# ethz-asl/laser_slam

Measured on NVIDIA H100. Metric: ICP registrations/s (131072-pt scan vs 524288-pt map, 30 iterations), higher is better.
Workload: dtype f32

## Files before the change

laser_slam_b200/csrc/ls_grid.cuh:

```cuda
#pragma once
#include <cfloat>
#include <climits>
#include <cstring>

#include <vector_types.h>
#include <vector_functions.h>

#include "ls_math.cuh"

#define LS_FB 8
#define LS_FB3 (LS_FB * LS_FB * LS_FB)
#define LS_PYR_LEVELS 7

namespace ls {

struct Entry {
  uint32_t start;
  int32_t meta;
};

struct Grid {
  float org[3];
  float H0, H1;
  float inv0, inv1;
  int dim[3];
  int n_cells0;
  float margin;
  float mu[3];
  int m;
  int leaf_split;
  int n_tab1;
  int overflow;
  int n_pyr;
  int pdim[LS_PYR_LEVELS + 1][3];
  int poff[LS_PYR_LEVELS + 1];
  int n_pyr_cells;
};

struct GridView {
  const Entry* top;
  const Entry* tab1;
  const float4* pts;
  const unsigned long long* pyr;
  const unsigned long long* topmask;
};

struct Best {
  float d2;
  int idx;
  int pos;
  LS_HD float bound() const { return d2; }
  LS_HD void offer(float d, int i, int p) {
    if (d < d2 || (d == d2 && i < idx)) {
      d2 = d;
      idx = i;
      pos = p;
    }
  }
  LS_HD void offer_pt(float d, const float4& c, int p);
};

#define LS_KNN_MAX 16
struct TopK {
  float d[LS_KNN_MAX];
  int id[LS_KNN_MAX];
  int k;
  float cap;
  LS_HD void reset(int kk) {
    k = kk;
    cap = INFINITY;
    for (int j = 0; j < LS_KNN_MAX; ++j) { d[j] = INFINITY; id[j] = INT_MAX; }
  }
  LS_HD float bound() const { return fminf(d[k - 1], cap); }
  LS_HD void offer(float dist, int i, int) {
    if (dist > cap || !(dist < d[k - 1] || (dist == d[k - 1] && i < id[k - 1]))) return;
    for (int j = 0; j < k; ++j)
      if (id[j] == i) return;
    int j = k - 1;
    while (j > 0 && (dist < d[j - 1] || (dist == d[j - 1] && i < id[j - 1]))) {
      d[j] = d[j - 1];
      id[j] = id[j - 1];
      --j;
    }
    d[j] = dist;
    id[j] = i;
  }
  LS_HD void offer_pt(float dist, const float4& c, int p);
};

#if defined(LS_SIM_COUNTERS) && !defined(__CUDA_ARCH__)
extern thread_local long long ls_sim_cand, ls_sim_entries, ls_sim_steps;
#define LS_CNT_CAND() (++ls_sim_cand)
#define LS_CNT_ENTRY() (++ls_sim_entries)
#define LS_CNT_STEP() (++ls_sim_steps)
#else
#define LS_CNT_CAND() ((void)0)
#define LS_CNT_ENTRY() ((void)0)
#define LS_CNT_STEP() ((void)0)
#endif

#if defined(__CUDA_ARCH__)
LS_HD float4 ld_pt(const float4* p) { return __ldg(p); }
LS_HD Entry ld_entry(const Entry* e) {
  const int2 v = __ldg(reinterpret_cast<const int2*>(e));
  Entry r;
  r.start = (uint32_t)v.x;
  r.meta = v.y;
  return r;
}
LS_HD int f2i(float f) { return __float_as_int(f); }
LS_HD float i2f(int i) { return __int_as_float(i); }
LS_HD float4 ld_state4(const float4* p) { return __ldcg(p); }
LS_HD void st_state4(float4* p, const float4 v) { __stcg(p, v); }
LS_HD unsigned long long ld_mask(const unsigned long long* p) { return __ldg(p); }
LS_HD unsigned long long ld_rows(const unsigned long long* p) { return __ldg(p); }
LS_HD int ctz64(unsigned long long m) { return __ffsll((long long)m) - 1; }
#else
LS_HD float4 ld_pt(const float4* p) { LS_CNT_CAND(); return *p; }
LS_HD Entry ld_entry(const Entry* e) { LS_CNT_ENTRY(); return *e; }
LS_HD int f2i(float f) { int i; std::memcpy(&i, &f, 4); return i; }
LS_HD float i2f(int i) { float f; std::memcpy(&f, &i, 4); return f; }
LS_HD float4 ld_state4(const float4* p) { return *p; }
LS_HD void st_state4(float4* p, const float4 v) { *p = v; }
LS_HD unsigned long long ld_mask(const unsigned long long* p) { LS_CNT_ENTRY(); return *p; }
LS_HD unsigned long long ld_rows(const unsigned long long* p) { return *p; }
LS_HD int ctz64(unsigned long long m) { return __builtin_ctzll(m); }
#endif

LS_HD int coord_top(float v, float o, float inv, int n) {
  float t = floorf((v - o) * inv);
  t = fminf(fmaxf(t, 0.0f), (float)(n - 1));
  return (int)t;
}
LS_HD int coord_sub(float v, float lo, float inv) {
  float t = floorf((v - lo) * inv);
  t = fminf(fmaxf(t, 0.0f), (float)(LS_FB - 1));
  return (int)t;
}
LS_HD float cell_lo(float o, int c, float H) { return o + (float)c * H; }

LS_HD float gap(float q, float lo, float hi, float m) {
  const float a = (lo - m) - q;
  const float b = q - (hi + m);
  return fmaxf(0.0f, fmaxf(a, b));
}

#define LS_SHRINK 0.999999f

LS_HD float ball_radius(float best_d2, float margin) { return sqrtf(best_d2) * 1.000001f + margin; }

LS_HD void Best::offer_pt(float d, const float4& c, int p) { offer(d, f2i(c.w), p); }
LS_HD void TopK::offer_pt(float dist, const float4& c, int p) { offer(dist, f2i(c.w), p); }
template <class Acc>
LS_HD void consider_pt(const float4 p, int pos, float qx, float qy, float qz, Acc& b) {
  b.offer_pt(dist2(qx, qy, qz, p.x, p.y, p.z), p, pos);
}
template <class Acc>
LS_HD void consider(const float4* pts, int pos, float qx, float qy, float qz, Acc& b) {
  consider_pt(ld_pt(pts + pos), pos, qx, qy, qz, b);
}

template <class Acc>
LS_HD void scan_range(const float4* pts, uint32_t a, uint32_t e, float qx, float qy, float qz, Acc& b) {
  uint32_t pos = a;
  for (; pos + 4 <= e; pos += 4) {
    LS_CNT_STEP();
    const float4 p0 = ld_pt(pts + pos), p1 = ld_pt(pts + pos + 1), p2 = ld_pt(pts + pos + 2), p3 = ld_pt(pts + pos + 3);
    consider_pt(p0, (int)pos, qx, qy, qz, b);
    consider_pt(p1, (int)pos + 1, qx, qy, qz, b);
    consider_pt(p2, (int)pos + 2, qx, qy, qz, b);
    consider_pt(p3, (int)pos + 3, qx, qy, qz, b);
  }
  if (pos < e) LS_CNT_STEP();
  for (; pos < e; ++pos) consider(pts, (int)pos, qx, qy, qz, b);
}

template <class Acc>
LS_HD void visit_fine(const Grid& g, const Entry* tab, unsigned long long rows, float lox, float loy, float loz,
                      const float4* pts, float qx, float qy, float qz, Acc& b) {
  const float R = ball_radius(b.bound(), g.margin);
  const int x0 = coord_sub(qx - R, lox, g.inv1), x1 = coord_sub(qx + R, lox, g.inv1);
  const int y0 = coord_sub(qy - R, loy, g.inv1), y1 = coord_sub(qy + R, loy, g.inv1);
  const int z0 = coord_sub(qz - R, loz, g.inv1), z1 = coord_sub(qz + R, loz, g.inv1);
  for (int z = z0; z <= z1; ++z) {
    const float gz = gap(qz, cell_lo(loz, z, g.H1), cell_lo(loz, z + 1, g.H1), g.margin);
    const float gz2 = gz * gz;
    if (gz2 * LS_SHRINK > b.bound()) continue;
    const Entry* row = tab + (z * LS_FB + y0) * LS_FB;
    for (int y = y0; y <= y1; ++y, row += LS_FB) {
      if (!((rows >> (z * LS_FB + y)) & 1ull)) continue;
      const float gy = gap(qy, cell_lo(loy, y, g.H1), cell_lo(loy, y + 1, g.H1), g.margin);
      const float lb = gy * gy + gz2;
      if (lb * LS_SHRINK > b.bound()) continue;
      LS_CNT_STEP();
      const Entry e0 = ld_entry(row + x0);
      const Entry e1 = ld_entry(row + x1);
      scan_range(pts, e0.start, e1.start + (uint32_t)e1.meta, qx, qy, qz, b);
    }
  }
}

template <class Acc>
LS_HD void visit_top_entry(const Grid& g, const GridView& v, const Entry e, unsigned long long rows, float cx, float cy,
                           float cz, float qx, float qy, float qz, Acc& b) {
  if (e.meta > 0) {
    scan_range(v.pts, e.start, e.start + (uint32_t)e.meta, qx, qy, qz, b);
  } else if (e.meta < 0) {
    visit_fine(g, v.tab1 + (size_t)(~e.meta) * LS_FB3, rows, cx, cy, cz, v.pts, qx, qy, qz, b);
  }
}
template <class Acc>
LS_HD void visit_top_cell(const Grid& g, const GridView& v, int x, int y, int z, float cx, float cy, float cz, float qx,
                          float qy, float qz, Acc& b) {
  LS_CNT_STEP();
  const size_t ci = ((size_t)z * g.dim[1] + y) * g.dim[0] + x;
  const Entry e = ld_entry(v.top + ci);
  const unsigned long long rows = ld_rows(v.topmask + ci);
  visit_top_entry(g, v, e, rows, cx, cy, cz, qx, qy, qz, b);
}

template <class Acc>
LS_HDN void pyramid_query(const Grid& g, const GridView& v, float qx, float qy, float qz, Acc& b) {
  int lvl[LS_PYR_LEVELS + 1], bx[LS_PYR_LEVELS + 1], by[LS_PYR_LEVELS + 1], bz[LS_PYR_LEVELS + 1];
  unsigned long long mk[LS_PYR_LEVELS + 1];
  const int* td = g.pdim[g.n_pyr];
  const int n_top = td[0] * td[1] * td[2];
  for (int t = 0; t < n_top; ++t) {
    int sp = 0;
    lvl[0] = g.n_pyr;
    bx[0] = (t % td[0]) * 4;
    by[0] = ((t / td[0]) % td[1]) * 4;
    bz[0] = (t / (td[0] * td[1])) * 4;
    mk[0] = ld_mask(v.pyr + g.poff[g.n_pyr] + t);
    while (sp >= 0) {
      if (mk[sp] == 0ull) { --sp; continue; }
      const int bit = ctz64(mk[sp]);
      mk[sp] &= mk[sp] - 1ull;
      LS_CNT_STEP();
      const int cl = lvl[sp] - 1;
      const int cx = bx[sp] + (bit & 3), cy = by[sp] + ((bit >> 2) & 3), cz = bz[sp] + (bit >> 4);
      const float Hc = g.H0 * (float)(1 << (2 * cl));
      const float lx = cell_lo(g.org[0], cx, Hc), ly = cell_lo(g.org[1], cy, Hc), lz = cell_lo(g.org[2], cz, Hc);
      const float gx = gap(qx, lx, cell_lo(g.org[0], cx + 1, Hc), g.margin);
      const float gy = gap(qy, ly, cell_lo(g.org[1], cy + 1, Hc), g.margin);
      const float gz = gap(qz, lz, cell_lo(g.org[2], cz + 1, Hc), g.margin);
      const float lb = gx * gx + (gy * gy + gz * gz);
      if (lb * LS_SHRINK > b.bound()) continue;
      if (cl == 0) {
        visit_top_cell(g, v, cx, cy, cz, lx, ly, lz, qx, qy, qz, b);
      } else {
        ++sp;
        lvl[sp] = cl;
        bx[sp] = cx * 4; by[sp] = cy * 4; bz[sp] = cz * 4;
        mk[sp] = ld_mask(v.pyr + g.poff[cl] + ((size_t)cz * g.pdim[cl][1] + cy) * g.pdim[cl][0] + cx);
      }
    }
  }
}

template <class Acc>
LS_HD void ball_query(const Grid& g, const GridView& v, float qx, float qy, float qz, Acc& b) {
  const float R = ball_radius(b.bound(), g.margin);
  const int x0 = coord_top(qx - R, g.org[0], g.inv0, g.dim[0]), x1 = coord_top(qx + R, g.org[0], g.inv0, g.dim[0]);
  const int y0 = coord_top(qy - R, g.org[1], g.inv0, g.dim[1]), y1 = coord_top(qy + R, g.org[1], g.inv0, g.dim[1]);
  const int z0 = coord_top(qz - R, g.org[2], g.inv0, g.dim[2]), z1 = coord_top(qz + R, g.org[2], g.inv0, g.dim[2]);
  if ((x1 - x0 + 1) * (y1 - y0 + 1) * (z1 - z0 + 1) > 27 && g.n_pyr > 0) {
    pyramid_query(g, v, qx, qy, qz, b);
    return;
  }
  for (int z = z0; z <= z1; ++z) {
    const float cz = cell_lo(g.org[2], z, g.H0);
    const float gz = gap(qz, cz, cell_lo(g.org[2], z + 1, g.H0), g.margin);
    const float gz2 = gz * gz;
    if (gz2 * LS_SHRINK > b.bound()) continue;
    for (int y = y0; y <= y1; ++y) {
      const float cy = cell_lo(g.org[1], y, g.H0);
      const float gy = gap(qy, cy, cell_lo(g.org[1], y + 1, g.H0), g.margin);
      const float lbyz = gy * gy + gz2;
      if (lbyz * LS_SHRINK > b.bound()) continue;
      for (int x = x0; x <= x1; ++x) {
        const float cx = cell_lo(g.org[0], x, g.H0);
        const float gx = gap(qx, cx, cell_lo(g.org[0], x + 1, g.H0), g.margin);
        const float lb = gx * gx + lbyz;
        if (lb * LS_SHRINK > b.bound()) continue;
        visit_top_cell(g, v, x, y, z, cx, cy, cz, qx, qy, qz, b);
      }
    }
  }
}

LS_HDN void seed_query(const Grid& g, const GridView& v, float qx, float qy, float qz, Best& b) {
  const int cx = coord_top(qx, g.org[0], g.inv0, g.dim[0]);
  const int cy = coord_top(qy, g.org[1], g.inv0, g.dim[1]);
  const int cz = coord_top(qz, g.org[2], g.inv0, g.dim[2]);
  const Entry e = ld_entry(v.top + ((size_t)cz * g.dim[1] + cy) * g.dim[0] + cx);
  if (e.meta == 0) {
    int X = 0, Y = 0, Z = 0;
    const int* td = g.pdim[g.n_pyr];
    const int n_top = td[0] * td[1] * td[2];
    if (n_top > 1) {
      const float Ht = g.H0 * (float)(1 << (2 * g.n_pyr));
      float best_lb = INFINITY;
      for (int t = 0; t < n_top; ++t) {
        if (ld_mask(v.pyr + g.poff[g.n_pyr] + t) == 0ull) continue;
        const int tx = t % td[0], ty = (t / td[0]) % td[1], tz = t / (td[0] * td[1]);
        const float gx = gap(qx, cell_lo(g.org[0], tx, Ht), cell_lo(g.org[0], tx + 1, Ht), 0.f);
        const float gy = gap(qy, cell_lo(g.org[1], ty, Ht), cell_lo(g.org[1], ty + 1, Ht), 0.f);
        const float gz = gap(qz, cell_lo(g.org[2], tz, Ht), cell_lo(g.org[2], tz + 1, Ht), 0.f);
        const float lb = gx * gx + (gy * gy + gz * gz);
        if (lb < best_lb) { best_lb = lb; X = tx; Y = ty; Z = tz; }
      }
    }
    for (int l = g.n_pyr; l >= 1; --l) {
      unsigned long long mask = ld_mask(v.pyr + g.poff[l] + ((size_t)Z * g.pdim[l][1] + Y) * g.pdim[l][0] + X);
      const float Hc = g.H0 * (float)(1 << (2 * (l - 1)));
      float best_lb = INFINITY;
      int best_bit = -1;
      while (mask) {
        const int bit = ctz64(mask);
        mask &= mask - 1ull;
        const int ccx = X * 4 + (bit & 3), ccy = Y * 4 + ((bit >> 2) & 3), ccz = Z * 4 + (bit >> 4);
        const float gx = gap(qx, cell_lo(g.org[0], ccx, Hc), cell_lo(g.org[0], ccx + 1, Hc), 0.f);
        const float gy = gap(qy, cell_lo(g.org[1], ccy, Hc), cell_lo(g.org[1], ccy + 1, Hc), 0.f);
        const float gz = gap(qz, cell_lo(g.org[2], ccz, Hc), cell_lo(g.org[2], ccz + 1, Hc), 0.f);
        const float lb = gx * gx + (gy * gy + gz * gz);
        if (lb < best_lb) { best_lb = lb; best_bit = bit; }
      }
      if (best_bit < 0) return;
      X = X * 4 + (best_bit & 3);
      Y = Y * 4 + ((best_bit >> 2) & 3);
      Z = Z * 4 + (best_bit >> 4);
    }
    const Entry s0 = ld_entry(v.top + ((size_t)Z * g.dim[1] + Y) * g.dim[0] + X);
    if (s0.meta != 0) consider(v.pts, (int)s0.start, qx, qy, qz, b);
    return;
  }
  if (e.meta > 0) { scan_range(v.pts, e.start, e.start + (uint32_t)e.meta, qx, qy, qz, b); return; }
  const float lox = cell_lo(g.org[0], cx, g.H0), loy = cell_lo(g.org[1], cy, g.H0), loz = cell_lo(g.org[2], cz, g.H0);
  const int fx = coord_sub(qx, lox, g.inv1), fy = coord_sub(qy, loy, g.inv1), fz = coord_sub(qz, loz, g.inv1);
  const Entry* tab = v.tab1 + (size_t)(~e.meta) * LS_FB3;
  const Entry e1 = ld_entry(tab + (fz * LS_FB + fy) * LS_FB + fx);
  if (e1.meta != 0) { scan_range(v.pts, e1.start, e1.start + (uint32_t)e1.meta, qx, qy, qz, b); return; }
  const int xa = fx > 0 ? fx - 1 : 0, xb = fx < LS_FB - 1 ? fx + 1 : LS_FB - 1;
  for (int z = (fz > 0 ? fz - 1 : 0); z <= (fz < LS_FB - 1 ? fz + 1 : LS_FB - 1); ++z)
    for (int y = (fy > 0 ? fy - 1 : 0); y <= (fy < LS_FB - 1 ? fy + 1 : LS_FB - 1); ++y) {
      const Entry r0 = ld_entry(tab + (z * LS_FB + y) * LS_FB + xa);
      const Entry r1 = ld_entry(tab + (z * LS_FB + y) * LS_FB + xb);
      scan_range(v.pts, r0.start, r1.start + (uint32_t)r1.meta, qx, qy, qz, b);
    }
  if (b.pos < 0) consider(v.pts, (int)e.start, qx, qy, qz, b);
}

LS_HD Best nn_search(const Grid& g, const GridView& v, float qx, float qy, float qz, int warm_pos, float cap_d2) {
  Best b;
  b.d2 = cap_d2;
  b.idx = INT_MAX;
  b.pos = -1;
  if (g.m <= 0) { b.idx = -1; b.d2 = INFINITY; return b; }
  if (warm_pos >= 0) consider(v.pts, warm_pos, qx, qy, qz, b);
  else seed_query(g, v, qx, qy, qz, b);
  ball_query(g, v, qx, qy, qz, b);
  if (b.pos < 0) { b.idx = -1; b.d2 = INFINITY; }
  return b;
}

#ifndef LS_VK
#define LS_VK 8
#endif
static_assert(LS_VK <= 15, "the list header keeps the candidate count in 4 bits");
#ifndef LS_VL_ABS
#define LS_VL_ABS 0.0f
#endif
#ifndef LS_VL_REL
#define LS_VL_REL 0.5f
#endif
#ifndef LS_VL_SKIN
#define LS_VL_SKIN 4.0f
#endif
#ifndef LS_VL_GATE
#define LS_VL_GATE 1.0f
#endif
struct VLists {
  float4* vq;
  float4* vpts;
  int n;
};

struct Collector {
  float r2;
  int cnt;
  float4* out;
  int stride;
  LS_HD float bound() const { return r2; }
  LS_HD void offer_pt(float d, const float4& c, int p) {
    if (d <= r2) {
      if (cnt < LS_VK) st_state4(out + (size_t)cnt * stride, make_float4(c.x, c.y, c.z, i2f(p)));
      else r2 = -1.0f;
      ++cnt;
    }
  }
};

LS_HD bool vlist_query(const VLists& L, const float4* pts, int i, const float4 v, const float4 c0, float qx, float qy,
                       float qz, float cap_d2, Best& b, float4& cbest) {
  const unsigned int bits = (unsigned int)f2i(v.w);
  if (bits == 0u) return false;
  const int cnt = (int)(bits & 15u);
  const float Rv = i2f((int)(bits & ~15u));
  const float Rc = Rv * 0.999996f - sqrtf(dist2(qx, qy, qz, v.x, v.y, v.z)) * 1.000004f;
  if (!(Rc > 0.0f)) return false;
  b.d2 = cap_d2;
  b.idx = INT_MAX;
  b.pos = -1;
  auto take = [&](const float4 c) {
    const float d = dist2(qx, qy, qz, c.x, c.y, c.z);
    const int cpos = f2i(c.w);
    if (d < b.d2) {
      b.d2 = d;
      b.pos = cpos;
      cbest = c;
    } else if (d == b.d2) {
      if (b.pos < 0 || f2i(ld_pt(pts + cpos).w) < f2i(ld_pt(pts + b.pos).w)) {
        b.pos = cpos;
        cbest = c;
      }
    }
  };
  if (cnt > 0) take(c0);
  for (int k0 = 1; k0 < cnt; k0 += 4) {
    float4 cs[4];
#pragma unroll
    for (int u = 0; u < 4; ++u)
      cs[u] = k0 + u < cnt ? ld_state4(L.vpts + (size_t)(k0 + u) * L.n + i) : make_float4(0.f, 0.f, 0.f, 0.f);
#pragma unroll
    for (int u = 0; u < 4; ++u)
      if (k0 + u < cnt) take(cs[u]);
  }
  return b.d2 * 1.00001f <= Rc * Rc;
}

LS_HD void vlist_build(const Grid& g, const GridView& v, const VLists& L, int i, float qx, float qy, float qz, bool found,
                       float found_d2, float cap_d2, float motion) {
  float Rv;
  if (found) {
    const float want = sqrtf(found_d2);
    const float margin = fmaxf(want * LS_VL_REL, LS_VL_ABS) + 1e-4f;
    if (!(motion * LS_VL_GATE <= margin)) return;
    Rv = want + fminf(margin, fmaxf(0.002f, LS_VL_SKIN * motion));
  } else {
    const float want = sqrtf(cap_d2);
    if (!(motion <= want * 0.125f)) return;
    Rv = want * 1.05f + fminf(want * 0.25f, fmaxf(0.002f, 4.0f * motion));
  }
  if (!(Rv < 3.0e38f)) return;
  Collector c;
  c.r2 = Rv * Rv;
  c.cnt = 0;
  c.out = L.vpts + i;
  c.stride = L.n;
  ball_query(g, v, qx, qy, qz, c);
  float4 head = make_float4(qx, qy, qz, 0.0f);
  if (c.cnt <= LS_VK) head.w = i2f((int)((((unsigned int)f2i(Rv * 0.9999999f)) & ~15u) | (unsigned int)c.cnt));
  st_state4(L.vq + i, head);
}

LS_HDN void knn_search(const Grid& g, const GridView& v, float qx, float qy, float qz, int k, TopK& t) {
  t.reset(k);
  if (g.m <= 0) return;
  const float extent = g.H0 * (float)(g.dim[0] + g.dim[1] + g.dim[2]) + 1.0f;
  float R = g.H1;
  for (int round = 0; round < 64; ++round) {
    t.cap = R * R;
    ball_query(g, v, qx, qy, qz, t);
    if (t.d[k - 1] <= t.cap) break;
    if (R > extent + fabsf(qx - g.org[0]) + fabsf(qy - g.org[1]) + fabsf(qz - g.org[2])) break;
    R = R * 2.0f;
  }
}

LS_HD int top_index(const Grid& g, float x, float y, float z) {
  const int cx = coord_top(x, g.org[0], g.inv0, g.dim[0]);
  const int cy = coord_top(y, g.org[1], g.inv0, g.dim[1]);
  const int cz = coord_top(z, g.org[2], g.inv0, g.dim[2]);
  return (cz * g.dim[1] + cy) * g.dim[0] + cx;
}
LS_HD void top_origin(const Grid& g, int c0, float& lox, float& loy, float& loz) {
  const int cx = c0 % g.dim[0];
  const int cy = (c0 / g.dim[0]) % g.dim[1];
  const int cz = c0 / (g.dim[0] * g.dim[1]);
  lox = cell_lo(g.org[0], cx, g.H0);
  loy = cell_lo(g.org[1], cy, g.H0);
  loz = cell_lo(g.org[2], cz, g.H0);
}
LS_HD int sub_index(float x, float y, float z, float lox, float loy, float loz, float inv) {
  return (coord_sub(z, loz, inv) * LS_FB + coord_sub(y, loy, inv)) * LS_FB + coord_sub(x, lox, inv);
}

LS_HDN void grid_setup(Grid& g, const float* lo, const float* hi, float cell_size, int max_cells, int leaf_split,
                       int m) {
  float H = cell_size > 0.f ? cell_size : 2.0f;
  float ext[3], emax = 0.f, oabs = 0.f;
  for (int a = 0; a < 3; ++a) {
    ext[a] = hi[a] - lo[a];
    if (!(ext[a] >= 0.f)) ext[a] = 0.f;
    emax = fmaxf(emax, ext[a]);
    oabs = fmaxf(oabs, fmaxf(fabsf(lo[a]), fabsf(hi[a])));
  }
  for (int it = 0; it < 40; ++it) {
    const float inv = 1.0f / H;
    double cells = 1.0;
    for (int a = 0; a < 3; ++a) cells *= (double)floorf(ext[a] * inv) + 1.0;
    if (cells <= (double)max_cells) break;
    H = H * 2.0f;
  }
  g.H0 = H;
  g.H1 = H / (float)LS_FB;
  g.inv0 = 1.0f / g.H0;
  g.inv1 = 1.0f / g.H1;
  int n = 1;
  for (int a = 0; a < 3; ++a) {
    g.org[a] = lo[a];
    int d = (int)floorf(ext[a] * g.inv0) + 1;
    if (d < 1) d = 1;
    g.dim[a] = d;
    n *= d;
  }
  g.n_cells0 = n;
  g.margin = (oabs + emax + H) * 1.9073486328125e-06f;
  g.m = m;
  g.leaf_split = leaf_split > 0 ? leaf_split : 32;
  g.n_tab1 = 0;
  g.overflow = 0;
  for (int a = 0; a < 3; ++a) g.pdim[0][a] = g.dim[a];
  g.poff[0] = 0;
  int off = 0, l = 0;
  do {
    ++l;
    for (int a = 0; a < 3; ++a) g.pdim[l][a] = (g.pdim[l - 1][a] + 3) / 4;
    g.poff[l] = off;
    off += g.pdim[l][0] * g.pdim[l][1] * g.pdim[l][2];
  } while ((g.pdim[l][0] > 1 || g.pdim[l][1] > 1 || g.pdim[l][2] > 1) && l < LS_PYR_LEVELS);
  g.n_pyr = l;
  g.n_pyr_cells = off;
}

}
```

Measured before the change: 984.2.

## Search fine cells in expanding rings from query cell, scanning rows outward

Adds a near-first traversal for nearest-neighbour queries whose bound is still large. It visits the query's home top cell first. Inside fine subgrids it walks y/z rows in expanding rings and scans each x row outward from the query position in both directions, stopping early once the x-gap exceeds the shrinking bound. It also skips the seed query when a finite cap distance is given. The intent is to tighten the bound sooner and prune more points and cells. The cost is more complex control flow, extra divergence and possibly redundant entry loads.

```diff
diff --git a/laser_slam_b200/csrc/ls_grid.cuh b/laser_slam_b200/csrc/ls_grid.cuh
--- a/laser_slam_b200/csrc/ls_grid.cuh
+++ b/laser_slam_b200/csrc/ls_grid.cuh
@@ -173,6 +173,66 @@
   }
   if (pos < e) LS_CNT_STEP();
   for (; pos < e; ++pos) consider(pts, (int)pos, qx, qy, qz, b);
+}
+
+template <class Acc>
+LS_HD void scan_half_row(const Grid& g, const float4* pts, int pos, uint32_t n, int d, float lox, float lbyz, float qx,
+                         float qy, float qz, Acc& b) {
+  for (; n >= 4; n -= 4, pos += 4 * d) {
+    LS_CNT_STEP();
+    const float4 p0 = ld_pt(pts + pos), p1 = ld_pt(pts + pos + d), p2 = ld_pt(pts + pos + 2 * d), p3 = ld_pt(pts + pos + 3 * d);
+    consider_pt(p0, pos, qx, qy, qz, b);
+    consider_pt(p1, pos + d, qx, qy, qz, b);
+    consider_pt(p2, pos + 2 * d, qx, qy, qz, b);
+    consider_pt(p3, pos + 3 * d, qx, qy, qz, b);
+    const int c = coord_sub(p3.x, lox, g.inv1);
+    const float gx = fmaxf(0.0f, d > 0 ? (cell_lo(lox, c, g.H1) - g.margin) - qx : qx - (cell_lo(lox, c + 1, g.H1) + g.margin));
+    if ((gx * gx + lbyz) * LS_SHRINK > b.bound()) return;
+  }
+  if (n > 0) LS_CNT_STEP();
+  for (; n > 0; --n, pos += d) consider(pts, pos, qx, qy, qz, b);
+}
+
+LS_HD unsigned long long row_box(int y0, int y1, int z0, int z1) {
+  const unsigned long long ys = (unsigned long long)((0xFFu >> (LS_FB - 1 - (y1 - y0))) << y0);
+  return (ys * 0x0101010101010101ull) & ((~0ull >> (LS_FB * (LS_FB - 1 - (z1 - z0)))) << (LS_FB * z0));
+}
+
+template <class Acc>
+LS_HD void visit_fine_rings(const Grid& g, const Entry* tab, unsigned long long rows, float lox, float loy, float loz,
+                      const float4* pts, float qx, float qy, float qz, Acc& b) {
+  const int fx = coord_sub(qx, lox, g.inv1), fy = coord_sub(qy, loy, g.inv1), fz = coord_sub(qz, loz, g.inv1);
+  unsigned long long done = 0ull;
+  for (int r = 0; r < LS_FB; ++r) {
+    const float R = ball_radius(b.bound(), g.margin);
+    const int ya = coord_sub(qy - R, loy, g.inv1), yb = coord_sub(qy + R, loy, g.inv1);
+    const int za = coord_sub(qz - R, loz, g.inv1), zb = coord_sub(qz + R, loz, g.inv1);
+    const int y0 = ya > fy - r ? ya : fy - r, y1 = yb < fy + r ? yb : fy + r;
+    const int z0 = za > fz - r ? za : fz - r, z1 = zb < fz + r ? zb : fz + r;
+    if (y0 > fy || y1 < fy || z0 > fz || z1 < fz || (y0 > fy - r && y1 < fy + r && z0 > fz - r && z1 < fz + r)) break;
+    const unsigned long long box = row_box(y0, y1, z0, z1);
+    unsigned long long ring = rows & box & ~done;
+    done |= box;
+    while (ring) {
+      const int bit = ctz64(ring);
+      ring &= ring - 1ull;
+      const int z = bit / LS_FB, y = bit % LS_FB;
+      const float gy = gap(qy, cell_lo(loy, y, g.H1), cell_lo(loy, y + 1, g.H1), g.margin);
+      const float gz = gap(qz, cell_lo(loz, z, g.H1), cell_lo(loz, z + 1, g.H1), g.margin);
+      const float lbyz = gy * gy + gz * gz;
+      if (lbyz * LS_SHRINK > b.bound()) continue;
+      const float Rx = ball_radius(b.bound(), g.margin);
+      const int x0 = coord_sub(qx - Rx, lox, g.inv1), x1 = coord_sub(qx + Rx, lox, g.inv1);
+      const Entry* row = tab + bit * LS_FB;
+      LS_CNT_STEP();
+      const Entry el = ld_entry(row + x0);
+      const Entry eh = ld_entry(row + fx);
+      const Entry er = ld_entry(row + x1);
+      for (int d = 1; d >= -1; d -= 2)
+        scan_half_row(g, pts, d > 0 ? (int)eh.start : (int)eh.start - 1,
+                      d > 0 ? er.start + (uint32_t)er.meta - eh.start : eh.start - el.start, d, lox, lbyz, qx, qy, qz, b);
+    }
+  }
 }
 
 template <class Acc>
@@ -200,23 +260,24 @@
   }
 }
 
-template <class Acc>
+template <bool kRings, class Acc>
 LS_HD void visit_top_entry(const Grid& g, const GridView& v, const Entry e, unsigned long long rows, float cx, float cy,
                            float cz, float qx, float qy, float qz, Acc& b) {
   if (e.meta > 0) {
     scan_range(v.pts, e.start, e.start + (uint32_t)e.meta, qx, qy, qz, b);
   } else if (e.meta < 0) {
-    visit_fine(g, v.tab1 + (size_t)(~e.meta) * LS_FB3, rows, cx, cy, cz, v.pts, qx, qy, qz, b);
-  }
-}
-template <class Acc>
+    if constexpr (kRings) visit_fine_rings(g, v.tab1 + (size_t)(~e.meta) * LS_FB3, rows, cx, cy, cz, v.pts, qx, qy, qz, b);
+    else visit_fine(g, v.tab1 + (size_t)(~e.meta) * LS_FB3, rows, cx, cy, cz, v.pts, qx, qy, qz, b);
+  }
+}
+template <bool kRings, class Acc>
 LS_HD void visit_top_cell(const Grid& g, const GridView& v, int x, int y, int z, float cx, float cy, float cz, float qx,
                           float qy, float qz, Acc& b) {
   LS_CNT_STEP();
   const size_t ci = ((size_t)z * g.dim[1] + y) * g.dim[0] + x;
   const Entry e = ld_entry(v.top + ci);
   const unsigned long long rows = ld_rows(v.topmask + ci);
-  visit_top_entry(g, v, e, rows, cx, cy, cz, qx, qy, qz, b);
+  visit_top_entry<kRings>(g, v, e, rows, cx, cy, cz, qx, qy, qz, b);
 }
 
 template <class Acc>
@@ -247,7 +308,7 @@
       const float lb = gx * gx + (gy * gy + gz * gz);
       if (lb * LS_SHRINK > b.bound()) continue;
       if (cl == 0) {
-        visit_top_cell(g, v, cx, cy, cz, lx, ly, lz, qx, qy, qz, b);
+        visit_top_cell<false>(g, v, cx, cy, cz, lx, ly, lz, qx, qy, qz, b);
       } else {
         ++sp;
         lvl[sp] = cl;
@@ -283,9 +344,39 @@
         const float gx = gap(qx, cx, cell_lo(g.org[0], x + 1, g.H0), g.margin);
         const float lb = gx * gx + lbyz;
         if (lb * LS_SHRINK > b.bound()) continue;
-        visit_top_cell(g, v, x, y, z, cx, cy, cz, qx, qy, qz, b);
+        visit_top_cell<false>(g, v, x, y, z, cx, cy, cz, qx, qy, qz, b);
       }
     }
+  }
+}
+
+LS_HD void ball_query_near(const Grid& g, const GridView& v, float qx, float qy, float qz, Best& b) {
+  const float R = ball_radius(b.bound(), g.margin);
+  const int x0 = coord_top(qx - R, g.org[0], g.inv0, g.dim[0]), x1 = coord_top(qx + R, g.org[0], g.inv0, g.dim[0]);
+  const int y0 = coord_top(qy - R, g.org[1], g.inv0, g.dim[1]), y1 = coord_top(qy + R, g.org[1], g.inv0, g.dim[1]);
+  const int z0 = coord_top(qz - R, g.org[2], g.inv0, g.dim[2]), z1 = coord_top(qz + R, g.org[2], g.inv0, g.dim[2]);
+  if ((x1 - x0 + 1) * (y1 - y0 + 1) * (z1 - z0 + 1) > 27 && g.n_pyr > 0) {
+    pyramid_query(g, v, qx, qy, qz, b);
+    return;
+  }
+  const int hx = coord_top(qx, g.org[0], g.inv0, g.dim[0]);
+  const int hy = coord_top(qy, g.org[1], g.inv0, g.dim[1]);
+  const int hz = coord_top(qz, g.org[2], g.inv0, g.dim[2]);
+  const int nx = x1 - x0 + 1, nxy = nx * (y1 - y0 + 1);
+  for (int t = -1; t < nxy * (z1 - z0 + 1); ++t) {
+    int x = hx, y = hy, z = hz;
+    if (t >= 0) {
+      x = x0 + t % nx;
+      y = y0 + (t % nxy) / nx;
+      z = z0 + t / nxy;
+      if (x == hx && y == hy && z == hz) continue;
+    }
+    const float cx = cell_lo(g.org[0], x, g.H0), cy = cell_lo(g.org[1], y, g.H0), cz = cell_lo(g.org[2], z, g.H0);
+    const float gx = gap(qx, cx, cell_lo(g.org[0], x + 1, g.H0), g.margin);
+    const float gy = gap(qy, cy, cell_lo(g.org[1], y + 1, g.H0), g.margin);
+    const float gz = gap(qz, cz, cell_lo(g.org[2], z + 1, g.H0), g.margin);
+    if ((gx * gx + (gy * gy + gz * gz)) * LS_SHRINK > b.bound()) continue;
+    visit_top_cell<true>(g, v, x, y, z, cx, cy, cz, qx, qy, qz, b);
   }
 }
 
@@ -358,8 +449,9 @@
   b.pos = -1;
   if (g.m <= 0) { b.idx = -1; b.d2 = INFINITY; return b; }
   if (warm_pos >= 0) consider(v.pts, warm_pos, qx, qy, qz, b);
-  else seed_query(g, v, qx, qy, qz, b);
-  ball_query(g, v, qx, qy, qz, b);
+  else if (!(cap_d2 < INFINITY)) seed_query(g, v, qx, qy, qz, b);
+  if (b.bound() > g.H1 * g.H1) ball_query_near(g, v, qx, qy, qz, b);
+  else ball_query(g, v, qx, qy, qz, b);
   if (b.pos < 0) { b.idx = -1; b.d2 = INFINITY; }
   return b;
 }
```

Result: faster. 1006, median of 6 (+2.2%).
